# liortalker/MindTheEdge

Hardware: AMD Instinct MI355X
Metric: training images/sec, PackNet-SAN+edge-loss 384x1280 bf16 (higher is better)
Workload: dtype bf16; 1 GPU; T8: PackNet-SAN + silog + 4-scale depth-edge loss training step, 384x1280, 8 frames/GPU, dropout 0.5, flip 0.5; global_batch=8, height=384, width=1280, parallelism=single GPU

## Files before the change

### mindtheedge_amd/csrc/conv_igemm.hip

```cpp
#include "common.hpp"
#include "conv_args.hpp"

__attribute__((visibility("hidden"))) int wgrad9_launch(const void* x, long ldx, const void* dy, long ldy, float* dw_stage, int parts_cap, int* parts_out,
                                                        int B, int H, int W, int Cin_p, int N, hipStream_t st);

#ifdef MTE_STAMPS
__device__ unsigned long long g_igemm_stamps[16384 * 8];
extern "C" int mtei_igemm_stamps(unsigned long long* host, int n) {
    return hipMemcpyFromSymbol(host, HIP_SYMBOL(g_igemm_stamps), sizeof(unsigned long long) * n) == hipSuccess ? 0 : -1;
}
#endif

namespace {


template <typename T> struct Mma;
template <> struct Mma<bf16_t> {
    __device__ static __forceinline__ void run(const u32x4_t& a, const u32x4_t& b, f32x16_t& c) {
        c = __builtin_amdgcn_mfma_f32_32x32x16_bf16(__builtin_bit_cast(bf16x8_t, a), __builtin_bit_cast(bf16x8_t, b), c, 0, 0, 0);
    }
};
template <> struct Mma<float> {
    __device__ static __forceinline__ void run(const u32x4_t& a, const u32x4_t& b, f32x16_t& c) {
#pragma unroll
// ... 1262 lines not shown
                                                               int Cout, int Cin, int taps, int Cin_p) {
    extern __shared__ float s_w[];
    const int n = blockIdx.x, c0 = blockIdx.y * 64;
    const int nc = min(64, Cin - c0);
    const float* src = w + ((long)n * Cin + c0) * taps;
    for (int i = threadIdx.x; i < nc * taps; i += 256) s_w[i] = src[i];
    __syncthreads();
    const int ncp = min(64, Cin_p - c0);
    for (int i = threadIdx.x; i < taps * ncp; i += 256) {
        const int tap = i / ncp, cl = i - tap * ncp;
        Elem<T>::st(wf + ((long)n * taps + tap) * Cin_p + c0 + cl, cl < nc ? s_w[cl * taps + tap] : 0.f);
    }
}

template <typename T>
__global__ __launch_bounds__(256) void pack_weights_bwd_kernel(const T* __restrict__ wf, T* __restrict__ wb,
                                                               int Cout, int taps, int Cin_p, int Cout_p) {
    __shared__ T tile[64][64 + 2];
    const int Kp = taps * Cin_p;
    const int n0 = blockIdx.x * 64, k0 = blockIdx.y * 64;
    for (int i = threadIdx.x; i < 64 * 64; i += 256) {
        const int r = i >> 6, cidx = i & 63;
        const int n = n0 + r, k = k0 + cidx;
        tile[r][cidx] = (n < Cout && k < Kp) ? wf[(long)n * Kp + k] : (T)0;
    }
    __syncthreads();
    for (int i = threadIdx.x; i < 64 * 64; i += 256) {
        const int kk = i >> 6, nn = i & 63;
        const int k = k0 + kk, n = n0 + nn;
        if (k < Kp && n < Cout_p) {
            const int tap = k / Cin_p, c = k - tap * Cin_p;
            wb[((long)c * taps + (taps - 1 - tap)) * Cout_p + n] = n < Cout ? tile[nn][kk] : (T)0;
        }
    }
}

struct PackJob {
    const float* w;
    void* wf;
    void* wb;
    void* pf;
    void* pb;
    int Cout, Cin, taps, Cin_p;
    int end_f, end_b, end_pf, end_pb;
};
constexpr int PACK_JOBS_MAX = 48;
struct PackTable { int n; int pad_; PackJob j[PACK_JOBS_MAX]; };
constexpr int PACK_FRAG_PER_BLOCK = 256 * 8;

template <typename T> __device__ __forceinline__ void store8(T* dst, const float* v);
template <> __device__ __forceinline__ void store8<bf16_t>(bf16_t* dst, const float* v) { *(u32x4_t*)dst = pack16<bf16_t>(v); }
template <> __device__ __forceinline__ void store8<float>(float* dst, const float* v) {
    *(u32x4_t*)dst = pack16<float>(v); *(u32x4_t*)(dst + 4) = pack16<float>(v + 4);
}

__host__ __device__ inline int pack_fn(int taps) { const int f = (64 * 65) / (64 * taps); return f < 1 ? 1 : (f > 16 ? 16 : f); }

template <typename T>
__global__ __launch_bounds__(256) void pack_multi_kernel(const PackTable tb) {
    __shared__ float s_w[64 * 65];
    int ji = 0;
    while (ji + 1 < tb.n && (int)blockIdx.x >= tb.j[ji].end_pb) ++ji;
    const PackJob& J = tb.j[ji];
    const int start = ji ? tb.j[ji - 1].end_pb : 0;
    const int bid = blockIdx.x;
    const int Cout = J.Cout, Cin = J.Cin, taps = J.taps, Cin_p = J.Cin_p;
    const float* __restrict__ w = J.w;
    if (bid < J.end_f) {
        const int fn = pack_fn(taps);
        const int cchunks = (Cin_p + 63) >> 6;
        const int lb = bid - start, n0 = (lb / cchunks) * fn, c0 = (lb - (lb / cchunks) * cchunks) * 64;
        const int nc = min(64, Cin - c0), nn = min(fn, Cout - n0);
        const int run = nc > 0 ? nc * taps : 0, rs = 64 * taps;
        for (int i = threadIdx.x; i < nn * run; i += 256) {
            const int ni = i / run, r = i - ni * run;
            s_w[ni * rs + r] = w[((long)(n0 + ni) * Cin + c0) * taps + r];
        }
        __syncthreads();
        const int ncp = min(64, Cin_p - c0), nch = ncp >> 3;
        T* wf = (T*)J.wf;
        for (int i = threadIdx.x; i < nn * taps * nch; i += 256) {
            const int ch8 = i % nch, t2 = i / nch, tap = t2 % taps, ni = t2 / taps;
            float v[8];
#pragma unroll
            for (int j = 0; j < 8; ++j) {
                const int cl = ch8 * 8 + j;
                v[j] = cl < nc ? s_w[ni * rs + cl * taps + tap] : 0.f;
            }
            store8<T>(wf + ((long)(n0 + ni) * taps + tap) * Cin_p + c0 + ch8 * 8, v);
        }
        return;
    }
    if (bid < J.end_b) {
        const int Kp = taps * Cin_p, Kr = taps * Cin;
        const int ktiles = (Kp + 63) >> 6;
        const int lb = bid - J.end_f, n0 = (lb / ktiles) * 64, k0 = (lb % ktiles) * 64;
        for (int i = threadIdx.x; i < 64 * 64; i += 256) {
            const int r = i >> 6, kk = i & 63;
            const int n = n0 + r, k = k0 + kk;
            s_w[r * 65 + kk] = (n < Cout && k < Kr) ? w[(long)n * Kr + k] : 0.f;
        }
        __syncthreads();
        T* wb = (T*)J.wb;
        if (Cout % 8 == 0) {
            for (int i = threadIdx.x; i < 64 * 8; i += 256) {
                const int kk = i >> 3, n8 = i & 7;
                const int k = k0 + kk, n = n0 + n8 * 8;
                if (k < Kp && n < Cout) {
                    const int c = k / taps, tap = k - c * taps;
                    float v[8];
#pragma unroll
                    for (int j = 0; j < 8; ++j) v[j] = s_w[(n8 * 8 + j) * 65 + kk];
                    store8<T>(wb + ((long)c * taps + (taps - 1 - tap)) * Cout + n, v);
                }
            }
            return;
        }
        for (int i = threadIdx.x; i < 64 * 64; i += 256) {
            const int kk = i >> 6, nn = i & 63;
            const int k = k0 + kk, n = n0 + nn;
            if (k < Kp && n < Cout) {
                const int c = k / taps, tap = k - c * taps;
                Elem<T>::st(wb + ((long)c * taps + (taps - 1 - tap)) * Cout + n, s_w[nn * 65 + kk]);
            }
        }
        return;
    }
    const bool fwd = bid < J.end_pf;
    const int N = fwd ? Cout : Cin_p, C = fwd ? Cin_p : Cout;
    const int NT = (N + 31) >> 5;
    const long total8 = (long)((C + 31) >> 5) * taps * 2 * NT * 64;
    const long i8 = (long)(bid - (fwd ? J.end_b : J.end_pf)) * 256 + threadIdx.x;
    if (i8 >= total8) return;
    long t = i8;
    const int lane = (int)(t & 63); t >>= 6;
    const int nt = (int)(t % NT); t /= NT;
    const int kk = (int)(t & 1); t >>= 1;
    const int tap = (int)(t % taps); const int sl = (int)(t / taps);
    const int n = nt * 32 + (lane & 31), c0 = sl * 32 + kk * 16 + (lane >> 5) * 8;
    float v[8];
#pragma unroll
    for (int j = 0; j < 8; ++j) {
        const int c = c0 + j;
        float x = 0.f;
        if (n < N && c < C) {
            if (fwd) { if (c < Cin) x = w[((long)n * Cin + c) * taps + tap]; }
            else if (n < Cin) x = w[((long)c * Cin + n) * taps + (taps - 1 - tap)];
        }
        v[j] = x;
    }
    store8<T>((T*)(fwd ? J.pf : J.pb) + i8 * 8, v);
}

__global__ __launch_bounds__(256) void unpack_wgrad_kernel(const float* __restrict__ st, float* __restrict__ dw, int Cout, int Cin, int taps, int Cin_p, int parts) {
    extern __shared__ float s_t[];
    const int n = blockIdx.x, c0 = blockIdx.y * 64;
    const int nc = min(64, Cin - c0);
    if (nc <= 0) return;
    const float* src = st + (long)n * taps * Cin_p + c0;
    const long pstride = (long)Cout * taps * Cin_p;
    for (int i = threadIdx.x; i < taps * 16; i += 256) {
        const int tap = i >> 4, c4 = (i & 15) * 4;
        if (c0 + c4 >= Cin_p) continue;
        const float* q = src + (long)tap * Cin_p + c4;
        f32x4_t acc = {0.f, 0.f, 0.f, 0.f};
        int p = 0;
        for (; p + 8 <= parts; p += 8) {
            f32x4_t v[8];
#pragma unroll
            for (int k = 0; k < 8; ++k) v[k] = *(const f32x4_t*)(q + (long)(p + k) * pstride);
#pragma unroll
            for (int k = 0; k < 8; ++k) acc += v[k];
        }
        for (; p < parts; ++p) acc += *(const f32x4_t*)(q + (long)p * pstride);
#pragma unroll
        for (int e = 0; e < 4; ++e) s_t[tap * 65 + c4 + e] = acc[e];
    }
    __syncthreads();
    float* dst = dw + ((long)n * Cin + c0) * taps;
    for (int i = threadIdx.x; i < nc * taps; i += 256) {
        const int cl = i / taps, tap = i - cl * taps;
        dst[i] = s_t[tap * 65 + cl];
    }
}

constexpr int RP_PC = 16;
__global__ __launch_bounds__(256) void reduce_parts_kernel(float* __restrict__ st, long elems, int parts, int pc) {
    const long i4 = blockIdx.x * 256L + threadIdx.x;
    if (i4 * 4 >= elems) return;
    const int p0 = blockIdx.y * pc, p1 = min(parts, p0 + pc);
    f32x4_t acc = {0.f, 0.f, 0.f, 0.f};
    for (int q = p0; q < p1; q += RP_PC) {
        f32x4_t v[RP_PC];
#pragma unroll
        for (int k = 0; k < RP_PC; ++k)
            v[k] = q + k < p1 ? *(const f32x4_t*)(st + (long)(q + k) * elems + i4 * 4) : f32x4_t{0.f, 0.f, 0.f, 0.f};
#pragma unroll
        for (int k = 0; k < RP_PC; ++k) acc += v[k];
    }
    *(f32x4_t*)(st + ((long)parts + blockIdx.y) * elems + i4 * 4) = acc;
}

template <typename T>
__global__ __launch_bounds__(256) void colsum_kernel(const T* __restrict__ y, long ld, long M, int N, float* __restrict__ out) {
    constexpr int PER16 = Elem<T>::PER16;
    const int cpr = N / PER16;
    const int tid = threadIdx.x;
    float acc[PER16];
#pragma unroll
    for (int i = 0; i < PER16; ++i) acc[i] = 0.f;
    const int cc = tid % cpr;
    const int rlane = tid / cpr, rstep = 256 / cpr;
    extern __shared__ float s_col[];
    for (int i = tid; i < N; i += 256) s_col[i] = 0.f;
    __syncthreads();
    if (rlane < rstep) {
        for (long m = (long)blockIdx.x * rstep + rlane; m < M; m += (long)gridDim.x * rstep) {
            float v[PER16];
            unpack16<T>(*(const u32x4_t*)(y + m * ld + cc * PER16), v);
#pragma unroll
            for (int i = 0; i < PER16; ++i) acc[i] += v[i];
        }
#pragma unroll
        for (int i = 0; i < PER16; ++i) atomicAdd(&s_col[cc * PER16 + i], acc[i]);
    }
    __syncthreads();
    for (int i = tid; i < N; i += 256) atomicAdd(out + i, s_col[i]);
}

}

extern "C" {

#ifdef MTE_DEV
extern "C" int mtei_set_pack3d_lds(int value);
extern "C" int mtei_set_gn(int which, int value);
extern "C" int mtei_set_patch_tall(int v);
extern "C" int mtei_set_tap_wgrad(int v);
extern "C" int mtei_set_head_mfma(int v);
extern int g_wgrad9, g_wgrad9_wgs, g_igemm8_one;
int mte_debug_set(int key, int value) {
    if (key == 26) { g_wgrad9 = value; return MTE_OK; }
    if (key == 27) { g_wgrad9_wgs = value; return MTE_OK; }
    if (key == 28) { g_igemm8_one = value; return MTE_OK; }
    if (key == 30) return mtei_set_head_mfma(value);
    if (key == 31) return mtei_set_tap_wgrad(value);
    if (key == 0) { g_igemm_dma = value; return MTE_OK; }
    if (key == 1) return mtei_set_pack3d_lds(value);
    if (key == 2 || key == 3) return mtei_set_gn(key - 2, value);
    if (key == 13) return mtei_set_gn(2, value);
    if (key == 15) { g_igemm_ring6 = value; return MTE_OK; }
    if (key == 17) { g_igemm_ablate = value; return MTE_OK; }
    if (key == 19) { g_igemm_pair_ksteps = value; return MTE_OK; }
    if (key == 21) { g_igemm_pp = value; return MTE_OK; }
    if (key == 23) { g_igemm8 = value; return MTE_OK; }
    if (key == 24) { g_igemm8_min_tiles = value; return MTE_OK; }
    if (key == 29) { g_igemm8_split_bn128 = value; return MTE_OK; }
    if (key == 32) { g_igemm_n32_dma = value; return MTE_OK; }
    if (key == 14) return mtei_set_gn(3, value);
    if (key == 25) return mtei_set_gn(4, value);
    if (key == 4) { g_wgrad_dma = value; return MTE_OK; }
    if (key == 6) { g_igemm_big = value; return MTE_OK; }
    if (key == 8) { g_wgrad_big = value; return MTE_OK; }
    if (key == 9) { g_wgrad_wgs = value; return MTE_OK; }
    if (key == 11) return mtei_set_patch_tall(value);
    if (key == 7) { g_igemm_big_min_tiles = value; return MTE_OK; }
    return MTE_ERR_ARG;
}
#endif

int mte_conv2d_igemm(const void* x, long ldx, const void* wpack, const float* bias, void* y, long ldy, int out_f32,
                     int B, int H, int W, int Cin_p, int N, int KH, int KW, int dtype,
                     float* workspace, long workspace_elems, int accumulate, hipStream_t stream) {
    (void)hipGetLastError();
    if (!x || !wpack || !y || B <= 0 || H <= 0 || W <= 0 || N <= 0) return MTE_ERR_ARG;
    const int per16 = dtype == MTE_DT_BF16 ? 8 : 4;
    if (Cin_p % 8 != 0 || ldx % per16 != 0 || (KH & 1) == 0 || (KW & 1) == 0) return MTE_ERR_ARG;
    ConvArgs a{x, ldx, wpack, bias, y, ldy, out_f32, B, H, W, Cin_p, N, KH, KW, (long)B * H * W, 1, workspace, accumulate & 1, (accumulate >> 1) & 1,
               nullptr, nullptr};
    if (dtype == MTE_DT_BF16) return dispatch_igemm<bf16_t>(a, workspace_elems, stream);
    if (dtype == MTE_DT_F32) return dispatch_igemm<float>(a, workspace_elems, stream);
    return MTE_ERR_UNSUPPORTED;
}

int mte_conv2d_igemm_unshuffle(const void* x, long ldx, const void* wpack, void* y, long ldy,
                               int B, int H, int W, int Cin_p, int N, int KH, int KW, int dtype, int accumulate, hipStream_t stream) {
    (void)hipGetLastError();
    if (!x || !wpack || !y || B <= 0 || H <= 0 || W <= 0 || N <= 0) return MTE_ERR_ARG;
    if (dtype != MTE_DT_BF16) return MTE_ERR_UNSUPPORTED;
    if (Cin_p % 8 != 0 || ldx % 8 != 0 || ldy % 8 != 0 || (KH & 1) == 0 || (KW & 1) == 0 || N % 32 != 0) return MTE_ERR_ARG;
    ConvArgs a{x, ldx, wpack, nullptr, y, ldy, 0, B, H, W, Cin_p, N, KH, KW, (long)B * H * W, 1, nullptr, accumulate & 1, 0, nullptr, nullptr, 0, N / 4};
    if (!(g_igemm_dma == 1 && Cin_p % 32 == 0)) return MTE_ERR_UNSUPPORTED;
    return dispatch_igemm<bf16_t>(a, 0, stream);
}

int mte_conv2d_igemm_sparse(const void* x, long ldx, const void* wpack, const float* bias, void* y, long ldy,
                            int B, int H, int W, int Cin_p, int N, int KH, int KW, int dtype,
                            const int* sites, const int* count, int accumulate, hipStream_t stream) {
    (void)hipGetLastError();
    if (!x || !wpack || !y || !sites || !count || B <= 0 || H <= 0 || W <= 0 || N <= 0 || (long)B * H * W > 0x7fffffffL) return MTE_ERR_ARG;
    const int per16 = dtype == MTE_DT_BF16 ? 8 : 4;
    if (Cin_p % 8 != 0 || ldx % per16 != 0 || (KH & 1) == 0 || (KW & 1) == 0) return MTE_ERR_ARG;
    ConvArgs a{x, ldx, wpack, bias, y, ldy, 0, B, H, W, Cin_p, N, KH, KW, (long)B * H * W, 1, nullptr, accumulate & 1, (accumulate >> 1) & 1,
               sites, count};
    if (dtype == MTE_DT_BF16) return dispatch_igemm<bf16_t>(a, 0, stream);
    if (dtype == MTE_DT_F32) return dispatch_igemm<float>(a, 0, stream);
    return MTE_ERR_UNSUPPORTED;
}

int mte_conv2d_wgrad(const void* x, long ldx, const void* dy, long ldy, float* dw_stage, int stage_parts, int* parts_out,
                     int B, int H, int W, int Cin_p, int N, int KH, int KW, int dtype, hipStream_t stream) {
    (void)hipGetLastError();
    if (!x || !dy || !dw_stage) return MTE_ERR_ARG;
    if (Cin_p % 8 != 0 || N % 8 != 0) return MTE_ERR_ARG;
    WgradArgs a{x, ldx, dy, ldy, dw_stage, B, H, W, Cin_p, N, KH, KW, (long)B * H * W, 1, 0, 0, 0};
    if (dtype == MTE_DT_BF16 && KH == 3 && KW == 3 && stage_parts >= 1 && parts_out) {
        const int rc = wgrad9_launch(x, ldx, dy, ldy, dw_stage, stage_parts, parts_out, B, H, W, Cin_p, N, stream);
        if (rc != MTE_ERR_UNSUPPORTED) return rc;
    }
    if (dtype == MTE_DT_BF16) return dispatch_wgrad<bf16_t>(a, stream, stage_parts, parts_out);
    if (dtype == MTE_DT_F32) return dispatch_wgrad<float>(a, stream, stage_parts, parts_out);
    return MTE_ERR_UNSUPPORTED;
}

int mte_pack_conv_weights(const float* w_oihw, void* wfwd, void* wbwd, int Cout, int Cin, int KH, int KW,
                          int Cin_p, int Cout_p, int dtype, hipStream_t stream) {
    (void)hipGetLastError();
    if (!w_oihw || !wfwd) return MTE_ERR_ARG;
    const int taps = KH * KW;
    if (Cout_p != Cout && wbwd) return MTE_ERR_ARG;
    const dim3 gf(Cout, (Cin_p + 63) / 64), gb((Cout + 63) / 64, (taps * Cin_p + 63) / 64);
    const size_t lds = sizeof(float) * 64 * taps;
    if (dtype == MTE_DT_BF16) {
        hipLaunchKernelGGL(pack_weights_fwd_kernel<bf16_t>, gf, dim3(256), lds, stream, w_oihw, (bf16_t*)wfwd, Cout, Cin, taps, Cin_p);
        if (wbwd) hipLaunchKernelGGL(pack_weights_bwd_kernel<bf16_t>, gb, dim3(256), 0, stream, (const bf16_t*)wfwd, (bf16_t*)wbwd, Cout, taps, Cin_p, Cout_p);
    } else {
        hipLaunchKernelGGL(pack_weights_fwd_kernel<float>, gf, dim3(256), lds, stream, w_oihw, (float*)wfwd, Cout, Cin, taps, Cin_p);
        if (wbwd) hipLaunchKernelGGL(pack_weights_bwd_kernel<float>, gb, dim3(256), 0, stream, (const float*)wfwd, (float*)wbwd, Cout, taps, Cin_p, Cout_p);
    }
    return mte_check_launch();
}

int mte_pack_conv_weights_multi(const void* jobs_host, int njobs, int dtype, hipStream_t stream) {
    (void)hipGetLastError();
    if (!jobs_host || njobs < 0 || (dtype != MTE_DT_BF16 && dtype != MTE_DT_F32)) return MTE_ERR_ARG;
    const PackJob* src = (const PackJob*)jobs_host;
    for (int j0 = 0; j0 < njobs; j0 += PACK_JOBS_MAX) {
        PackTable tb{};
        tb.n = njobs - j0 < PACK_JOBS_MAX ? njobs - j0 : PACK_JOBS_MAX;
        long blocks = 0;
        for (int i = 0; i < tb.n; ++i) {
            PackJob J = src[j0 + i];
            if (!J.w || !J.wf || J.taps < 1 || J.taps > 49 || J.Cin_p % 8 != 0 || J.Cin > J.Cin_p) return MTE_ERR_ARG;
            if ((J.pf || J.pb) && dtype != MTE_DT_BF16) return MTE_ERR_ARG;
            if (J.pb && !J.wb) return MTE_ERR_ARG;
            blocks += (long)((J.Cout + pack_fn(J.taps) - 1) / pack_fn(J.taps)) * ((J.Cin_p + 63) / 64);
            J.end_f = (int)blocks;
            if (J.wb) blocks += (long)((J.Cout + 63) / 64) * ((J.taps * J.Cin_p + 63) / 64);
            J.end_b = (int)blocks;
            if (J.pf) blocks += ((long)((J.Cin_p + 31) / 32) * J.taps * 2 * ((J.Cout + 31) / 32) * 64 + 255) / 256;
            J.end_pf = (int)blocks;
            if (J.pb) blocks += ((long)((J.Cout + 31) / 32) * J.taps * 2 * ((J.Cin_p + 31) / 32) * 64 + 255) / 256;
            J.end_pb = (int)blocks;
            if (blocks > 0x7fffffffL) return MTE_ERR_UNSUPPORTED;
            tb.j[i] = J;
        }
        if (blocks == 0) continue;
        if (dtype == MTE_DT_BF16) hipLaunchKernelGGL(pack_multi_kernel<bf16_t>, dim3((unsigned)blocks), dim3(256), 0, stream, tb);
        else hipLaunchKernelGGL(pack_multi_kernel<float>, dim3((unsigned)blocks), dim3(256), 0, stream, tb);
    }
    return mte_check_launch();
}

int mte_pack_conv_weights_bwd(const void* wfwd, void* wbwd, int Cout, int KH, int KW, int Cin_p, int dtype, hipStream_t stream) {
    (void)hipGetLastError();
    if (!wfwd || !wbwd) return MTE_ERR_ARG;
    const int taps = KH * KW;
    const dim3 gb((Cout + 63) / 64, (taps * Cin_p + 63) / 64);
    if (dtype == MTE_DT_BF16) hipLaunchKernelGGL(pack_weights_bwd_kernel<bf16_t>, gb, dim3(256), 0, stream, (const bf16_t*)wfwd, (bf16_t*)wbwd, Cout, taps, Cin_p, Cout);
    else hipLaunchKernelGGL(pack_weights_bwd_kernel<float>, gb, dim3(256), 0, stream, (const float*)wfwd, (float*)wbwd, Cout, taps, Cin_p, Cout);
    return mte_check_launch();
}

int mte_unpack_conv_wgrad(float* dw_stage, int parts, float* dw_oihw, int Cout, int Cin, int KH, int KW, int Cin_p, hipStream_t stream) {
    (void)hipGetLastError();
    if (!dw_stage || !dw_oihw || parts < 1) return MTE_ERR_ARG;
    const dim3 grid(Cout, (Cin + 63) / 64);
    if (parts > 32) {
        const long elems = (long)Cout * KH * KW * Cin_p;
        const int pc = ((parts + 31) / 32 + RP_PC - 1) / RP_PC * RP_PC;
        const int groups = (parts + pc - 1) / pc;
        hipLaunchKernelGGL(reduce_parts_kernel, dim3((unsigned)((elems / 4 + 255) / 256), (unsigned)groups), dim3(256), 0, stream, dw_stage, elems, parts, pc);
        dw_stage += (long)parts * elems;
        parts = groups;
    }
    hipLaunchKernelGGL(unpack_wgrad_kernel, grid, dim3(256), sizeof(float) * KH * KW * 65, stream, dw_stage, dw_oihw, Cout, Cin, KH * KW, Cin_p, parts);
    return mte_check_launch();
}

int mte_colsum(const void* y, long ld, long M, int N, float* out, int dtype, hipStream_t stream) {
    (void)hipGetLastError();
    if (!y || !out || N % 8 != 0) return MTE_ERR_ARG;
    const int per16 = dtype == MTE_DT_BF16 ? 8 : 4;
    if (N / per16 > 256) return MTE_ERR_UNSUPPORTED;
    if (mte_memset_async(out, 0, sizeof(float) * N, stream) != hipSuccess) return MTE_ERR_LAUNCH;
    const int rstep = 256 / (N / per16);
    long want = (M + rstep - 1) / rstep;
    want = (want + 31) / 32;
    const int grid = (int)(want > 1024 ? 1024 : (want < 1 ? 1 : want));
    if (dtype == MTE_DT_BF16) hipLaunchKernelGGL(colsum_kernel<bf16_t>, dim3(grid), dim3(256), sizeof(float) * N, stream, (const bf16_t*)y, ld, M, N, out);
    else hipLaunchKernelGGL(colsum_kernel<float>, dim3(grid), dim3(256), sizeof(float) * N, stream, (const float*)y, ld, M, N, out);
    return mte_check_launch();
}

}
```

### mindtheedge_amd/kernels.py

```python
import ctypes
import itertools
import math
import os
import weakref

import torch

from ._lib import lib, MteError

DT_BF16, DT_F32 = 0, 1
_state = {"compute_dtype": torch.bfloat16, "weights_epoch": 0}


def set_compute_dtype(dtype):
    dtype = {"bf16": torch.bfloat16, "fp32": torch.float32, "f32": torch.float32}.get(dtype, dtype)
    assert dtype in (torch.bfloat16, torch.float32)
    _state["compute_dtype"] = dtype


def compute_dtype():
    return _state["compute_dtype"]


def bump_weights_epoch():
# ... 490 lines not shown

class SiteList:

    def __init__(self, mask):
        _require_gpu(mask)
        if mask.dtype != torch.uint8 or not mask.is_contiguous():
            raise MteError("site list: expected a contiguous uint8 mask [B,H,W]")
        n = mask.numel()
        self.rows = torch.empty((n,), dtype=torch.int32, device=mask.device)
        self.count = torch.empty((1,), dtype=torch.int32, device=mask.device)
        ws = torch.empty((int(lib.mte_sparse_site_list_workspace_elems(n)),), dtype=torch.int32, device=mask.device)
        lib.mte_sparse_site_list(mask.data_ptr(), n, self.rows.data_ptr(), self.count.data_ptr(), ws.data_ptr(), _stream())
        self.shape = tuple(mask.shape)


def conv_forward(x, wf, bias, cout, kh, kw, out=None, pack=None, w=None, accumulate=False, sites=None, gn_records=None):
    B, Cp, H, W = x.shape
    if out is None:
        out = new_act(B, cout, H, W, x.dtype, x.device)
        if sites is not None:
            out.zero_()
    xp, ldx = _pl(x)
    yp, ldy = _pl(out)
    if sites is not None:
        if sites.shape != (B, H, W):
            raise MteError("site list of a %s mask used on a %s map" % (sites.shape, (B, H, W)))
        lib.mte_conv2d_igemm_sparse(xp, ldx, wf.data_ptr(), _ptr(bias), yp, ldy, B, H, W, Cp, cout, kh, kw, _dt(x),
                                    sites.rows.data_ptr(), sites.count.data_ptr(), 1 if accumulate else 0, _stream())
        return out
    if not accumulate and _stem_ok(W, Cp, cout, kh, kw, x.dtype):
        lib.mte_conv2d_stem_fwd(xp, ldx, wf.data_ptr(), _ptr(bias), yp, ldy, B, H, W, cout, kh, kw, _stream())
        return out
    if pack is not None and _patch_ok(W, Cp, cout, kh, kw, x.dtype):
        if (gn_records is not None and _cfg["gn_stats_in_conv"] and cout % 16 == 0
                and lib.mte_gn_fwd_is_single_pass_b(B, H * W, cout, 0, _dt(x)) != 1):
            n = int(lib.mte_conv2d_patch_fwd_gn_elems(B, H, W))
            rec = torch.empty((n,), dtype=torch.float32, device=x.device)
            tiles = ctypes.c_int(0)
            lib.mte_conv2d_patch_fwd_gn(xp, ldx, pack.get_patch(w, 'f').data_ptr(), _ptr(bias), yp, ldy, B, H, W, Cp, cout, kh, kw,
                                        1 if accumulate else 0, rec.data_ptr(), n, ctypes.byref(tiles), _stream())
            gn_records.append((rec, tiles.value))
            return out
        lib.mte_conv2d_patch_fwd(xp, ldx, pack.get_patch(w, 'f').data_ptr(), _ptr(bias), yp, ldy, B, H, W, Cp, cout, kh, kw,
                                 1 if accumulate else 0, _stream())
        return out
    ws, ws_n = _splitk_workspace(B * H * W, cout, x.device)
    lib.mte_conv2d_igemm(xp, ldx, wf.data_ptr(), _ptr(bias), yp, ldy, 0, B, H, W, Cp, cout, kh, kw, _dt(x), _ptr(ws), ws_n,
                         (1 if accumulate else 0) | _CONV_SOLO, _stream())
    return out


_CONV_SOLO = 2


_side = {"enabled": True, "streams": [], "next": 0, "keep": [], "keep_bytes": 0, "callback_queued": False, "dirty": False}
lib.set_option(3, 1, lazy=True)
def _new_side_stream():
    pr = int(os.environ.get("MTE_SIDE_PRIORITY", "1"))
    if pr == 0:
        return torch.cuda.Stream()
    hip = ctypes.CDLL("libamdhip64.so")
    h = ctypes.c_void_p()
    if hip.hipStreamCreateWithPriority(ctypes.byref(h), 1, pr) != 0:
        raise RuntimeError("hipStreamCreateWithPriority(%d) failed" % pr)
    return torch.cuda.ExternalStream(h.value)


_SIDE_STREAMS = 1
_SIDE_KEEP_LIMIT = 24 << 30


def use_wgrad_side_stream(flag):
    _side["enabled"] = bool(flag)
    lib.set_option(3, 1 if flag else 0, lazy=True)


class _BandChain:

    def __enter__(self):
        return self

    def __exit__(self, *exc):
        return False

    def mark(self):
        return None

    def join(self, ev=None):
        return None


def join_side_stream():
    if _side["dirty"]:
        for st in _side["streams"]:
            ev = torch.cuda.Event()
            ev.record(st)
            torch.cuda.current_stream().wait_event(ev)
        _side["dirty"] = False
    _side["keep"].clear()
    _side["keep_bytes"] = 0


def side_streams_wait_into(stream):
    if _side["dirty"]:
        for st in _side["streams"]:
            ev = torch.cuda.Event()
            ev.record(st)
            stream.wait_event(ev)


def _side_join_callback():
    _side["callback_queued"] = False
    join_side_stream()


def _side_stream_for(*tensors):
    if not _side["streams"]:
        _side["streams"] = [_new_side_stream() for _ in range(max(1, _SIDE_STREAMS))]
    side = _side["streams"][_side["next"] % len(_side["streams"])]
    _side["next"] += 1
    ev = torch.cuda.Event()
    ev.record()
    side.wait_event(ev)
    _side["keep"].append(tensors)
    _side["keep_bytes"] += sum(t.numel() * t.element_size() for t in tensors)
    _side["dirty"] = True
    if not _side["callback_queued"]:
        try:
            torch.autograd.Variable._execution_engine.queue_callback(_side_join_callback)
            _side["callback_queued"] = True
        except RuntimeError:
            pass
    return side


def _conv_wgrad(x, dy, w, need_dbias, dw_out, dbias_out):
    cout, cin, kh, kw = w.shape
    B, Cp, H, W = x.shape
    dyp, lddy = _pl(dy)
    xp, ldx = _pl(x)
    st = _stream()
    dbias = None
    per = cout * kh * kw * Cp
    patch = _cfg["patch_kernels"] and x.dtype == torch.bfloat16 and lib.mte_conv2d_patch_wgrad_supported(W, Cp, cout, kh, kw, DT_BF16) == 1
    if patch and lib.mte_conv2d_wgrad_nine_tap(H, W, Cp, cout, kh, kw, _dt(x)) == 1:
        patch = False
    if kh * kw == 1 and Cp >= 64:
        patch = False
    wide = 256 if per <= (1 << 18) else (64 if per <= (1 << 19) else 32)
    cap = max(1, min(512, (192 << 20) // (4 * per))) if patch and _cfg["patch_wgrad_slabs"] else max(1, min(wide, (96 << 20) // (4 * per)))
    stem = _stem_ok(W, Cp, cout, kh, kw, x.dtype)
    if stem:
        cap = 2048
    stage = torch.empty((cap + (32 if cap > 32 else 0), cout, kh * kw, Cp), dtype=torch.float32, device=x.device)
    parts = ctypes.c_int(1)
    if stem:
        lib.mte_conv2d_stem_wgrad(xp, ldx, dyp, lddy, stage.data_ptr(), cap, ctypes.byref(parts), B, H, W, cout, kh, kw, st)
    elif patch:
        lib.mte_conv2d_patch_wgrad(xp, ldx, dyp, lddy, stage.data_ptr(), cap, ctypes.byref(parts), B, H, W, Cp, cout, kh, kw, st)
    else:
        lib.mte_conv2d_wgrad(xp, ldx, dyp, lddy, stage.data_ptr(), cap, ctypes.byref(parts), B, H, W, Cp, cout, kh, kw, _dt(x), st)
    dw = dw_out if dw_out is not None else torch.empty_like(w, dtype=torch.float32)
    lib.mte_unpack_conv_wgrad(stage.data_ptr(), parts.value, dw.data_ptr(), cout, cin, kh, kw, Cp, st)
    if need_dbias:
        dbias = dbias_out if dbias_out is not None else torch.empty((cout,), dtype=torch.float32, device=x.device)
        lib.mte_colsum(dyp, lddy, B * H * W, cout, dbias.data_ptr(), _dt(dy), st)
    return dw, dbias


def conv_backward(x, dy, w, pack, need_dx, need_dw=True, need_dbias=True, dw_out=None, dbias_out=None, fork_slot=None, sunk=False, sites=None):
    dw = dbias = dx = None
    on_side = False
    if need_dw:
        sunk = bool(sunk) and dw_out is not None and (dbias_out is not None or not need_dbias)
        on_side = sunk and _side["enabled"] and need_dx

    def wgrad():
        if on_side:
            if _side["keep_bytes"] > _SIDE_KEEP_LIMIT:
                join_side_stream()
            with torch.cuda.stream(_side_stream_for(x, dy)):
                return _conv_wgrad(x, dy, w, need_dbias, dw_out, dbias_out)
        return _conv_wgrad(x, dy, w, need_dbias, dw_out, dbias_out)

    if need_dw:
        dw, dbias = wgrad()
    if need_dx:
        dx = _conv_dgrad(x, dy, w, pack, fork_slot, sites)
    return dx, dw, dbias


def _conv_dgrad(x, dy, w, pack, fork_slot, sites):
    cout, cin, kh, kw = w.shape
    B, Cp, H, W = x.shape
    dyp, lddy = _pl(dy)
    st = _stream()
    target = _fork_target(fork_slot, (B, Cp, H, W), x.dtype, keep_pending=True)
    if (target is None and fork_slot is not None and (kh, kw) == (1, 1) and sites is None and _cfg["fold_shortcut_dgrad"]
            and not _cfg.get("no_fork_accumulate") and _patch_ok(W, cout, Cp, 1, 1, x.dtype) and _patch_ok(W, 32, Cp, 3, 3, x.dtype)):
        dx = new_act(B, Cp, H, W, x.dtype, x.device)
        fork_slot["buf"] = dx
        fork_slot["pending"] = (dy, w, pack)
        return dx
    pend = _pending_slot(fork_slot) if target is not None else None
    if pend is not None:
        dy3, w3, pack3 = pend["pending"]
        if ((kh, kw) == (3, 3) and sites is None and target is pend["buf"] and _patch_ok(W, cout, Cp, 3, 3, x.dtype)
                and tuple(dy3.shape[2:]) == (H, W) and dy3.dtype == x.dtype):
            del pend["pending"]
            d3p, ldd3 = _pl(dy3)
            dxp, lddx = _pl(target)
            lib.mte_conv2d_patch_fwd_plus1x1(dyp, lddy, pack.get_patch(w, 'b').data_ptr(), 0, dxp, lddx, B, H, W, cout, Cp,
                                             d3p, ldd3, pack3.get_patch(w3, 'b').data_ptr(), dy3.shape[1], st)
            fork_slot["buf"] = target
            return target
        _flush_pending(pend)
    dx = target if target is not None else new_act(B, Cp, H, W, x.dtype, x.device)
    if target is None and sites is not None:
        dx.zero_()
    acc = 1 if target is not None else 0
    dxp, lddx = _pl(dx)
    if sites is not None:
        _, wb = pack.get(w, x.dtype, True)
        lib.mte_conv2d_igemm_sparse(dyp, lddy, wb.data_ptr(), 0, dxp, lddx, B, H, W, cout, Cp, kh, kw, _dt(x),
                                    sites.rows.data_ptr(), sites.count.data_ptr(), acc, st)
    elif _patch_ok(W, cout, Cp, kh, kw, x.dtype):
        lib.mte_conv2d_patch_fwd(dyp, lddy, pack.get_patch(w, 'b').data_ptr(), 0, dxp, lddx, B, H, W, cout, Cp, kh, kw, acc, st)
    else:
        _, wb = pack.get(w, x.dtype, True)
        ws, ws_n = _splitk_workspace(B * H * W, Cp, x.device)
        lib.mte_conv2d_igemm(dyp, lddy, wb.data_ptr(), 0, dxp, lddx, 0, B, H, W, cout, Cp, kh, kw, _dt(x), _ptr(ws), ws_n, acc, st)
    if fork_slot is not None:
        fork_slot["buf"] = dx
    return dx


_stats_elems = {}


def gn_stats_buffer(B, device):
    n = _stats_elems.get(B)
    if n is None:
        n = _stats_elems[B] = int(lib.mte_gn_stats_elems(B))
    return _zeros((n,), torch.float64, device)


def _gn_forward(y1, y2, scale2, gamma, beta, eps, out=None, records=None):
    B, C, H, W = y1.shape
    p1, l1 = _pl(y1)
    p2, l2 = _pl(y2) if y2 is not None else (0, 0)
    st = _stream()
    ready = 1
    stats = gn_stats_buffer(B, y1.device)
    if lib.mte_gn_fwd_is_single_pass_b(B, H * W, C, 1 if y2 is not None else 0, _dt(y1)) == 1:
        ready = 0
    elif records and y2 is None:
        lib.mte_gn_stats_from_records(records[0][0].data_ptr(), records[0][1], stats.data_ptr(), B, st)
    else:
        lib.mte_gn_stats(p1, l1, p2, l2, _ptr(scale2), stats.data_ptr(), B, H * W, C, _dt(y1), st)
    z = out if out is not None else new_act(B, C, H, W, y1.dtype, y1.device)
    if tuple(z.shape) != (B, C, H, W) or z.dtype != y1.dtype:
        raise MteError("output destination has shape %s / %s, expected %s / %s" % (tuple(z.shape), z.dtype, (B, C, H, W), y1.dtype))
    zp, lz = _pl(z)
    lib.mte_gn_elu_fwd(p1, l1, p2, l2, _ptr(scale2), stats.data_ptr(), ready, gamma.data_ptr(), beta.data_ptr(), zp, lz,
                       B, H * W, C, eps, _dt(y1), st)
    return z, stats


def _gn_backward(dz, y1, y2, scale2, stats, gamma, beta, eps, need_d2, want_dbias=False, dgamma=None, dbeta=None, dbias=None):
    B, C, H, W = y1.shape
    dz = as_act(dz, y1.dtype)
    red = _zeros((B, C, 2), torch.float32, y1.device)
    d1 = new_act(B, C, H, W, y1.dtype, y1.device)
    d2 = new_act(B, C, H, W, y1.dtype, y1.device) if need_d2 else None
    dgamma = dgamma if dgamma is not None else _zeros((C,), torch.float32, y1.device)
    dbeta = dbeta if dbeta is not None else _zeros((C,), torch.float32, y1.device)
    if want_dbias and dbias is None:
        dbias = _zeros((C,), torch.float32, y1.device)
    pz, lz = _pl(dz)
    p1, l1 = _pl(y1)
    p2, l2 = _pl(y2) if y2 is not None else (0, 0)
    pd1, ld1 = _pl(d1)
    pd2, ld2 = _pl(d2) if d2 is not None else (0, 0)
    lib.mte_gn_elu_bwd(pz, lz, p1, l1, p2, l2, _ptr(scale2), stats.data_ptr(), gamma.data_ptr(), beta.data_ptr(), red.data_ptr(),
                       pd1, ld1, pd2, ld2, dgamma.data_ptr(), dbeta.data_ptr(), _ptr(dbias), B, H * W, C, eps, _dt(y1), _stream())
    if want_dbias:
        return d1, d2, dgamma, dbeta, dbias
    return d1, d2, dgamma, dbeta


GN_EPS = 1e-5

_dropout_pool = {}


def dropout2d_scale(B, C, p, device):
    key = (str(device), float(p))
    pool = _dropout_pool.get(key)
    n = B * C
    if pool is None or pool[1] + n > pool[0].numel():
        size = max(1 << 17, 2 * n)
        pool = _dropout_pool[key] = [(torch.rand((size,), device=device) >= p).float() / (1.0 - p), 0]
    out = pool[0][pool[1]:pool[1] + n].view(B, C)
    pool[1] += n
    return out


# ... 801 lines not shown
```

Baseline: 372.7 images/sec.

## Rework weight-gradient partial reduction into a split-K finish kernel with in-place staging

Replaces the separate reduce_parts + unpack_wgrad kernels with a single finish kernel. It splits the partial-sum reduction across several lanes per block and optionally across z-slices, writing slice sums back in place into the stage buffer before a second pass transposes to OIHW. Channel tile width adapts to Cin_p and to the needed parallelism. The extra 32-slot stage padding is dropped. The aim is more parallelism and less memory traffic when many partials exist, at the cost of more complex indexing and shared-memory use.

```diff
diff --git a/mindtheedge_amd/csrc/conv_igemm.hip b/mindtheedge_amd/csrc/conv_igemm.hip
--- a/mindtheedge_amd/csrc/conv_igemm.hip
+++ b/mindtheedge_amd/csrc/conv_igemm.hip
@@ -1438,53 +1438,82 @@
     store8<T>((T*)(fwd ? J.pf : J.pb) + i8 * 8, v);
 }
 
-__global__ __launch_bounds__(256) void unpack_wgrad_kernel(const float* __restrict__ st, float* __restrict__ dw, int Cout, int Cin, int taps, int Cin_p, int parts) {
+__global__ __launch_bounds__(256) void finish_wgrad_kernel(float* st, float* __restrict__ dw, int Cin, int taps, int Cin_p, int parts, long pstride,
+                                                           int S, int ccl, int PL, int to_stage) {
     extern __shared__ float s_t[];
-    const int n = blockIdx.x, c0 = blockIdx.y * 64;
-    const int nc = min(64, Cin - c0);
-    if (nc <= 0) return;
-    const float* src = st + (long)n * taps * Cin_p + c0;
-    const long pstride = (long)Cout * taps * Cin_p;
-    for (int i = threadIdx.x; i < taps * 16; i += 256) {
-        const int tap = i >> 4, c4 = (i & 15) * 4;
+    const int CC = 1 << ccl, items = taps << (ccl - 2), W = CC + 1, lsz = taps * W;
+    const int n = blockIdx.x, c0 = blockIdx.y * CC;
+    const int nc = min(CC, Cin - c0);
+    const int p0 = blockIdx.z * S, np = min(S, parts - p0);
+    if (nc <= 0 || np <= 0) return;
+    const int PLe = min(PL, np);
+    float* base = st + (long)p0 * pstride + (long)n * taps * Cin_p + c0;
+    for (int i = threadIdx.x; i < items * PLe; i += 256) {
+        const int lane = i / items, it = i - lane * items;
+        const int tap = it >> (ccl - 2), c4 = (it & ((CC >> 2) - 1)) * 4;
         if (c0 + c4 >= Cin_p) continue;
-        const float* q = src + (long)tap * Cin_p + c4;
+        const float* q = base + (long)lane * pstride + (long)tap * Cin_p + c4;
+        const long ls = (long)PLe * pstride;
+        const int cnt = (np - lane + PLe - 1) / PLe;
         f32x4_t acc = {0.f, 0.f, 0.f, 0.f};
-        int p = 0;
-        for (; p + 8 <= parts; p += 8) {
+        for (int k0 = 0; k0 < cnt; k0 += 8) {
             f32x4_t v[8];
 #pragma unroll
-            for (int k = 0; k < 8; ++k) v[k] = *(const f32x4_t*)(q + (long)(p + k) * pstride);
+            for (int k = 0; k < 8; ++k) v[k] = k0 + k < cnt ? *(const f32x4_t*)(q + (k0 + k) * ls) : f32x4_t{0.f, 0.f, 0.f, 0.f};
 #pragma unroll
             for (int k = 0; k < 8; ++k) acc += v[k];
         }
-        for (; p < parts; ++p) acc += *(const f32x4_t*)(q + (long)p * pstride);
-#pragma unroll
-        for (int e = 0; e < 4; ++e) s_t[tap * 65 + c4 + e] = acc[e];
+        float* s = s_t + lane * lsz + tap * W + c4;
+#pragma unroll
+        for (int e = 0; e < 4; ++e) s[e] = acc[e];
     }
     __syncthreads();
+    if (to_stage) {
+        for (int it = threadIdx.x; it < items; it += 256) {
+            const int tap = it >> (ccl - 2), c4 = (it & ((CC >> 2) - 1)) * 4;
+            if (c0 + c4 >= Cin_p) continue;
+            f32x4_t a;
+#pragma unroll
+            for (int e = 0; e < 4; ++e) a[e] = s_t[tap * W + c4 + e];
+            for (int l = 1; l < PLe; ++l)
+#pragma unroll
+                for (int e = 0; e < 4; ++e) a[e] += s_t[l * lsz + tap * W + c4 + e];
+            *(f32x4_t*)(base + (long)tap * Cin_p + c4) = a;
+        }
+        return;
+    }
     float* dst = dw + ((long)n * Cin + c0) * taps;
     for (int i = threadIdx.x; i < nc * taps; i += 256) {
         const int cl = i / taps, tap = i - cl * taps;
-        dst[i] = s_t[tap * 65 + cl];
-    }
-}
-
-constexpr int RP_PC = 16;
-__global__ __launch_bounds__(256) void reduce_parts_kernel(float* __restrict__ st, long elems, int parts, int pc) {
-    const long i4 = blockIdx.x * 256L + threadIdx.x;
-    if (i4 * 4 >= elems) return;
-    const int p0 = blockIdx.y * pc, p1 = min(parts, p0 + pc);
-    f32x4_t acc = {0.f, 0.f, 0.f, 0.f};
-    for (int q = p0; q < p1; q += RP_PC) {
-        f32x4_t v[RP_PC];
-#pragma unroll
-        for (int k = 0; k < RP_PC; ++k)
-            v[k] = q + k < p1 ? *(const f32x4_t*)(st + (long)(q + k) * elems + i4 * 4) : f32x4_t{0.f, 0.f, 0.f, 0.f};
-#pragma unroll
-        for (int k = 0; k < RP_PC; ++k) acc += v[k];
-    }
-    *(f32x4_t*)(st + ((long)parts + blockIdx.y) * elems + i4 * 4) = acc;
+        float a = s_t[tap * W + cl];
+        for (int l = 1; l < PLe; ++l) a += s_t[l * lsz + tap * W + cl];
+        dst[i] = a;
+    }
+}
+
+inline int finish_lanes(int taps, int cc) { const int items = taps * cc / 4; return items >= 256 ? 1 : 256 / items; }
+
+inline int finish_want(int parts, long elems) {
+    const long w = ((9L << 20) + 32 * elems - 1) / (32 * elems);
+    const long cap = (parts + 7) / 8;
+    return (int)(w < cap ? w : cap);
+}
+
+inline int finish_slices(int parts, long elems, int taps) {
+    if (parts <= 64) return 1;
+    const int z = (finish_want(parts, elems) + finish_lanes(taps, 32) - 1) / finish_lanes(taps, 32);
+    return z > 8 ? 8 : z;
+}
+
+void launch_finish(float* st, long pstride, int parts, int S, int Z, float* dw, int Cout, int Cin, int taps, int Cin_p, hipStream_t stream) {
+    int ccl = 6;
+    while (ccl > 3 && (1 << (ccl - 1)) >= Cin_p) --ccl;
+    const int want = finish_want(parts, (long)Cout * taps * Cin_p);
+    while (ccl > 5 && finish_lanes(taps, 1 << ccl) * Z < want) --ccl;
+    const int CC = 1 << ccl, PL = finish_lanes(taps, CC);
+    const int lanes = PL < S ? PL : S;
+    hipLaunchKernelGGL(finish_wgrad_kernel, dim3(Cout, (Cin + CC - 1) / CC, Z), dim3(256), sizeof(float) * lanes * taps * (CC + 1), stream,
+                       st, dw, Cin, taps, Cin_p, parts, pstride, S, ccl, PL, Z > 1 ? 1 : 0);
 }
 
 template <typename T>
@@ -1670,17 +1699,18 @@
 
 int mte_unpack_conv_wgrad(float* dw_stage, int parts, float* dw_oihw, int Cout, int Cin, int KH, int KW, int Cin_p, hipStream_t stream) {
     (void)hipGetLastError();
-    if (!dw_stage || !dw_oihw || parts < 1) return MTE_ERR_ARG;
-    const dim3 grid(Cout, (Cin + 63) / 64);
-    if (parts > 32) {
-        const long elems = (long)Cout * KH * KW * Cin_p;
-        const int pc = ((parts + 31) / 32 + RP_PC - 1) / RP_PC * RP_PC;
-        const int groups = (parts + pc - 1) / pc;
-        hipLaunchKernelGGL(reduce_parts_kernel, dim3((unsigned)((elems / 4 + 255) / 256), (unsigned)groups), dim3(256), 0, stream, dw_stage, elems, parts, pc);
-        dw_stage += (long)parts * elems;
-        parts = groups;
-    }
-    hipLaunchKernelGGL(unpack_wgrad_kernel, grid, dim3(256), sizeof(float) * KH * KW * 65, stream, dw_stage, dw_oihw, Cout, Cin, KH * KW, Cin_p, parts);
+    if (!dw_stage || !dw_oihw || parts < 1 || Cout < 1 || Cin < 1 || Cin > Cin_p || Cin_p % 8 != 0 || KH * KW < 1 || KH * KW > 49) return MTE_ERR_ARG;
+    const int taps = KH * KW;
+    const long elems = (long)Cout * taps * Cin_p;
+    int Z = finish_slices(parts, elems, taps);
+    if (Z > 1) {
+        const int S = (parts + Z - 1) / Z;
+        Z = (parts + S - 1) / S;
+        launch_finish(dw_stage, elems, parts, S, Z, dw_oihw, Cout, Cin, taps, Cin_p, stream);
+        launch_finish(dw_stage, elems * S, Z, Z, 1, dw_oihw, Cout, Cin, taps, Cin_p, stream);
+    } else {
+        launch_finish(dw_stage, elems, parts, parts, 1, dw_oihw, Cout, Cin, taps, Cin_p, stream);
+    }
     return mte_check_launch();
 }
 
diff --git a/mindtheedge_amd/kernels.py b/mindtheedge_amd/kernels.py
--- a/mindtheedge_amd/kernels.py
+++ b/mindtheedge_amd/kernels.py
@@ -666,7 +666,7 @@
     stem = _stem_ok(W, Cp, cout, kh, kw, x.dtype)
     if stem:
         cap = 2048
-    stage = torch.empty((cap + (32 if cap > 32 else 0), cout, kh * kw, Cp), dtype=torch.float32, device=x.device)
+    stage = torch.empty((cap, cout, kh * kw, Cp), dtype=torch.float32, device=x.device)
     parts = ctypes.c_int(1)
     if stem:
         lib.mte_conv2d_stem_wgrad(xp, ldx, dyp, lddy, stage.data_ptr(), cap, ctypes.byref(parts), B, H, W, cout, kh, kw, st)
```

Result: no change. 374.6 images/sec, median of 6 (+0.5%).
